# knagrecha/saturn

Hardware: NVIDIA H100
Metric: candidate schedules/sec (higher is better)
Workload: dtype f32

## Files before the change

saturn_b200/csrc/sb_common.cuh:

```cuda
#pragma once
#include <cuda_runtime.h>
#include <stdint.h>

#include "../../include/saturn_b200.h"

#if defined(__CUDA_ARCH__) && (__CUDA_ARCH__ != 900)
#error "saturn_b200 kernels target sm_90a (H100) only"
#endif

namespace sb {

constexpr int kSlots = SB_NSLOT;
constexpr int kWarp = 32;
constexpr int kMaxNodes = SB_MAX_NODES;
constexpr float kSentinel = 1.0e6f;

__device__ __forceinline__ float inf_f() { return __int_as_float(0x7f800000); }

__device__ __forceinline__ uint32_t smem_u32(const void* p) {
  return static_cast<uint32_t>(__cvta_generic_to_shared(p));
}
__device__ __forceinline__ uint32_t cluster_ctarank() {
  uint32_t r;
  asm volatile("mov.u32 %0, %%cluster_ctarank;" : "=r"(r));
  return r;
}
__device__ __forceinline__ void cluster_sync_all() {
  asm volatile("barrier.cluster.arrive.release.aligned;" ::: "memory");
  asm volatile("barrier.cluster.wait.acquire.aligned;" ::: "memory");
}
__device__ __forceinline__ uint32_t cluster_map_shared(uint32_t addr, uint32_t rank) {
  uint32_t r;
  asm volatile("mapa.shared::cluster.u32 %0, %1, %2;" : "=r"(r) : "r"(addr), "r"(rank));
  return r;
}

__device__ __forceinline__ void mbar_init(uint64_t* bar, uint32_t count) {
  asm volatile("mbarrier.init.shared::cta.b64 [%0], %1;" ::"r"(smem_u32(bar)), "r"(count) : "memory");
}
__device__ __forceinline__ void mbar_fence_init() {
  asm volatile("fence.mbarrier_init.release.cluster;" ::: "memory");
}
__device__ __forceinline__ void fence_proxy_async() {
  asm volatile("fence.proxy.async.shared::cta;" ::: "memory");
}
__device__ __forceinline__ void mbar_arrive_expect_tx(uint64_t* bar, uint32_t bytes) {
  asm volatile("mbarrier.arrive.expect_tx.shared::cta.b64 _, [%0], %1;" ::"r"(smem_u32(bar)), "r"(bytes)
               : "memory");
}
__device__ __forceinline__ bool mbar_try_wait(uint64_t* bar, uint32_t parity) {
  uint32_t ok;
  asm volatile(
      "{\n\t.reg .pred p;\n\t"
      "mbarrier.try_wait.parity.shared::cta.b64 p, [%1], %2;\n\t"
      "selp.u32 %0, 1, 0, p;\n\t}"
      : "=r"(ok)
      : "r"(smem_u32(bar)), "r"(parity)
      : "memory");
  return ok != 0;
}
__device__ __forceinline__ void mbar_wait(uint64_t* bar, uint32_t parity) {
  uint32_t spins = 0;
  while (!mbar_try_wait(bar, parity)) {
    if (++spins > (1u << 26)) __trap();
  }
}
__device__ __forceinline__ void tma_bulk_g2s(void* dst_smem, const void* src_gmem, uint32_t bytes,
                                             uint64_t* bar) {
  asm volatile(
      "cp.async.bulk.shared::cluster.global.mbarrier::complete_tx::bytes [%0], [%1], %2, [%3];" ::"r"(
          smem_u32(dst_smem)),
      "l"(src_gmem), "r"(bytes), "r"(smem_u32(bar))
      : "memory");
}

__device__ __forceinline__ void pmov_fma(float& dst, float src, int bit, int one) {
  int d = __float_as_int(dst);
  asm("{\n\t.reg .pred p;\n\tsetp.ne.s32 p, %2, 0;\n\t@p mad.lo.s32 %0, %1, %3, 0;\n\t}"
      : "+r"(d)
      : "r"(__float_as_int(src)), "r"(bit), "r"(one));
  dst = __int_as_float(d);
}
__device__ __forceinline__ void pinf_fma(float& dst, int bit) {
  asm("{\n\t.reg .pred p;\n\tsetp.ne.s32 p, %1, 0;\n\t@p add.f32 %0, %0, 0f7F800000;\n\t}" : "+f"(dst) : "r"(bit));
}
__device__ __forceinline__ float psel(float a, float b, int bit) {
  float r;
  asm("{\n\t.reg .pred p;\n\tsetp.ne.s32 p, %3, 0;\n\tselp.f32 %0, %1, %2, p;\n\t}" : "=f"(r) : "f"(a), "f"(b), "r"(bit));
  return r;
}

__device__ __forceinline__ float fmax3_mk(float mk, float b, float c) {
  return __int_as_float(__vimax3_s32(__float_as_int(mk), __float_as_int(b), __float_as_int(c)));
}

template <bool kIntegerStarts, bool kTrackMk = kIntegerStarts, bool kSum = false, bool kWeighted = false,
          bool kDue = false>
__device__ __forceinline__ void ls_step(float (&f)[8], float& mk, float& pend, float rt, int km1, int one, int ph,
                                        float w = 0.f, float d = 0.f) {
  static_assert(kSum || !kWeighted, "weights scale the sum of completion times only");
  static_assert(kWeighted || !kDue, "due dates run on the weighted form (unit weights for plain tardiness)");
  const float INF = inf_f();
  const int b2 = km1 & 4, b1 = km1 & 2, b0 = km1 & 1;
  float x0 = psel(f[4], f[0], b2), x1 = psel(f[5], f[1], b2), x2 = psel(f[6], f[2], b2), x3 = psel(f[7], f[3], b2);
  const float m2 = psel(INF, -0.0f, b2);
  float x4 = f[4] + m2, x5 = f[5] + m2, x6 = f[6] + m2, x7 = f[7] + m2;
  pmov_fma(x0, x2, b1, one); pmov_fma(x1, x3, b1, one); pmov_fma(x2, x4, b1, one); pmov_fma(x3, x5, b1, one);
  pmov_fma(x4, x6, b1, one); pmov_fma(x5, x7, b1, one); pinf_fma(x6, b1); pinf_fma(x7, b1);
  pmov_fma(x0, x1, b0, one); pmov_fma(x1, x2, b0, one); pmov_fma(x2, x3, b0, one); pmov_fma(x3, x4, b0, one);
  pmov_fma(x4, x5, b0, one); pmov_fma(x5, x6, b0, one); pmov_fma(x6, x7, b0, one); pinf_fma(x7, b0);
  const float s = x0;
  float v;
  if (kIntegerStarts) {
    v = s + ceilf(rt);
  } else {
    v = s + rt;
  }
  if (kSum) {
    const float e = kIntegerStarts ? s + rt : v;
    if (kDue) mk = __fadd_rn(mk, __fmul_rn(w, fmaxf(__fsub_rn(e, d), 0.f)));
    else if (kWeighted) mk = __fadd_rn(mk, __fmul_rn(w, e));
    else mk = mk + e;
  } else if (kTrackMk) {
    const float e = kIntegerStarts ? s + rt : v;
    if (ph < 0) mk = fmaxf(mk, e);
    else if (ph == 0) pend = e;
    else mk = fmax3_mk(mk, pend, e);
  }
  f[0] = fmaxf(f[0], fminf(v, x1));
  f[1] = fmaxf(f[1], fminf(v, x2));
  f[2] = fmaxf(f[2], fminf(v, x3));
  f[3] = fmaxf(f[3], fminf(v, x4));
  f[4] = fmaxf(f[4], fminf(v, x5));
  f[5] = fmaxf(f[5], fminf(v, x6));
  f[6] = fmaxf(f[6], fminf(v, x7));
  f[7] = fmaxf(f[7], v);
}

__device__ __forceinline__ unsigned long long pack_key(float mk, uint32_t id) {
  return (static_cast<unsigned long long>(__float_as_uint(mk)) << 32) | id;
}

__device__ __host__ __forceinline__ uint64_t mix64(uint64_t z) {
  z += 0x9e3779b97f4a7c15ull;
  z = (z ^ (z >> 30)) * 0xbf58476d1ce4e5b9ull;
  z = (z ^ (z >> 27)) * 0x94d049bb133111ebull;
  return z ^ (z >> 31);
}
__device__ __host__ __forceinline__ uint64_t rng_u64(uint64_t seed, uint64_t stream, uint64_t ctr) {
  return mix64(mix64(seed ^ (stream * 0xd1342543de82ef95ull)) + ctr * 0x2545f4914f6cdd1dull);
}

}
```

saturn_b200/csrc/sb_eval.cu:

```cuda
#include "sb_lane.cuh"

namespace sb {

struct TileArgs {
  const float* tab;
  int J, SG;
  const uint8_t* opt;
  const uint8_t* prio;
  long long B;
  long long stride_o, stride_p;
  int row_o, row_p;
  int copy_o, copy_p;
  int use_bulk;
  int nodes;
  float* out;
  unsigned long long* best_key;
  uint32_t id_base;
  long long ntiles;
  int one;
  SearchFuse sf;
  XchgPost xp;
  const float* w;
  const float* d;
};

template <int PB, bool INT, bool STREAM, bool MULTI, bool SEARCH = false, bool TABG = false, int ADDR = 0,
          bool SUM = false, bool W = false, bool D = false>
__global__ void __launch_bounds__(STREAM ? 512 : 384, 1) k_eval_tiles(const TileArgs a) {
  static_assert(!(SEARCH && (STREAM || TABG)), "the fused search round runs on shared-memory tiles only");
  static_assert(ADDR == 0 || (!TABG && !MULTI && !SEARCH), "ADDR = 1 needs the table and the opt rows in shared memory");
  static_assert(SUM || !W, "weights scale the sum of completion times only");
  static_assert(W || !D, "due dates run on the weighted form");
  extern __shared__ __align__(128) uint8_t smem[];
  const int nw = blockDim.x >> 5;
  const int warp = threadIdx.x >> 5, lane = threadIdx.x & 31;
  const uint32_t tab_bytes = TABG ? 0u : static_cast<uint32_t>(a.J) * a.SG * 4u;
  const uint32_t w_bytes = (W && !TABG) ? ((static_cast<uint32_t>(a.J) * 4u + 15u) & ~15u) : 0u;
  const uint32_t d_bytes = D ? w_bytes : 0u;
  float* tab_s = reinterpret_cast<float*>(smem);
  [[maybe_unused]] float* w_s = reinterpret_cast<float*>(smem + tab_bytes);
  [[maybe_unused]] float* d_s = reinterpret_cast<float*>(smem + tab_bytes + w_bytes);
  uint64_t* bars = reinterpret_cast<uint64_t*>(smem + ((tab_bytes + w_bytes + d_bytes + 15u) & ~15u));
  uint8_t* tiles = reinterpret_cast<uint8_t*>(bars) + (((1 + nw) * 8 + 15) & ~15);
  const uint32_t node_bytes = MULTI ? static_cast<uint32_t>(a.nodes) * 1024u : 0u;
  const uint32_t tile_bytes = 32u * (a.row_o + (STREAM ? 0 : a.row_p)) + node_bytes;
  uint8_t* wbase = tiles + static_cast<size_t>(warp) * tile_bytes;
  float4* node_s = reinterpret_cast<float4*>(wbase);
  uint8_t* tile_o = wbase + node_bytes;
  uint8_t* tile_p = tile_o + 32u * a.row_o;
  uint64_t* bar_tab = bars;
  uint64_t* bar_w = bars + 1 + warp;

  if (threadIdx.x == 0) {
    mbar_init(bar_tab, 1);
    for (int w = 0; w < nw; ++w) mbar_init(bars + 1 + w, 1);
    mbar_fence_init();
  }
  __syncthreads();
  if constexpr (!TABG) {
    if (threadIdx.x == 0) {
      mbar_arrive_expect_tx(bar_tab, tab_bytes + w_bytes + d_bytes);
      const uint8_t* src = reinterpret_cast<const uint8_t*>(a.tab);
      for (uint32_t off = 0; off < tab_bytes; off += 32768u) {
        uint32_t n = min(32768u, tab_bytes - off);
        tma_bulk_g2s(smem + off, src + off, n, bar_tab);
      }
      if constexpr (W) {
        const uint8_t* wsrc = reinterpret_cast<const uint8_t*>(a.w);
        for (uint32_t off = 0; off < w_bytes; off += 32768u)
          tma_bulk_g2s(smem + tab_bytes + off, wsrc + off, min(32768u, w_bytes - off), bar_tab);
      }
      if constexpr (D) {
        const uint8_t* dsrc = reinterpret_cast<const uint8_t*>(a.d);
        for (uint32_t off = 0; off < d_bytes; off += 32768u)
          tma_bulk_g2s(smem + tab_bytes + w_bytes + off, dsrc + off, min(32768u, d_bytes - off), bar_tab);
      }
    }
  }

  LaneState<INT, MULTI, ADDR, SUM, (W ? (TABG ? 2 : 1) : 0), D> st;
  if (TABG) st.tab = a.tab;
  else st.tab = tab_s;
  if constexpr (W) {
    st.wt = TABG ? a.w : w_s;
    st.wt_s = smem_u32(w_s);
  }
  if constexpr (D) {
    st.dd = TABG ? a.d : d_s;
    st.dd_s = smem_u32(d_s);
  }
  st.SG = a.SG;
  st.one = a.one;
  st.orow = tile_o + lane * a.row_o;
  st.ns = node_s + lane;
  st.orow_s = smem_u32(tile_o + lane * a.row_o);
  st.tab_s = smem_u32(tab_s);
  st.four = static_cast<uint32_t>(a.one) * 4u;

  bool fold_pending = a.xp.counter != nullptr && a.xp.fold_prev && a.xp.seq > 1 && blockIdx.x == 0 && warp == 0;
  unsigned long long pf_seen = 0ull, pf_key = ~0ull;
  auto look_issue = [&]() {
    if (lane < a.xp.x.world) {
      const unsigned long long* slot = a.xp.x.peer[lane] + ((a.xp.seq - 1) & 1ull) * 2;
      asm volatile("ld.acquire.sys.global.u64 %0, [%1];" : "=l"(pf_seen) : "l"(slot + 1) : "memory");
      asm volatile("ld.relaxed.sys.global.u64 %0, [%1];" : "=l"(pf_key) : "l"(slot) : "memory");
    }
  };
  auto fold_keys = [&](unsigned long long k) {
#pragma unroll
    for (int d = 16; d > 0; d >>= 1) {
      const unsigned long long o = __shfl_xor_sync(0xffffffffu, k, d);
      k = o < k ? o : k;
    }
    if (lane == 0) atomicMin(a.best_key, k);
    fold_pending = false;
  };
  auto look_consume = [&]() {
    const unsigned long long want = a.xp.seq - 1;
    const bool ok = lane >= a.xp.x.world || pf_seen >= want;
    if (__all_sync(0xffffffffu, ok)) fold_keys(lane < a.xp.x.world ? pf_key : ~0ull);
  };
  auto try_fold = [&](bool block) {
    const unsigned long long want = a.xp.seq - 1;
    unsigned long long k = ~0ull;
    bool ok = true;
    if (lane < a.xp.x.world) {
      const unsigned long long* slot = a.xp.x.peer[lane] + (want & 1ull) * 2;
      unsigned long long seen;
      unsigned spins = 0;
      for (;;) {
        asm volatile("ld.acquire.sys.global.u64 %0, [%1];" : "=l"(seen) : "l"(slot + 1) : "memory");
        if (seen >= want || !block || ++spins >= (1u << 22)) break;
        __nanosleep(64);
      }
      ok = seen >= want;
      if (ok) asm volatile("ld.relaxed.sys.global.u64 %0, [%1];" : "=l"(k) : "l"(slot) : "memory");
    }
    ok = __all_sync(0xffffffffu, ok);
    if (!ok) {
      if (block && lane == 0) *a.xp.error = 1;
      return;
    }
    fold_keys(k);
  };
  if (fold_pending) look_issue();

  uint32_t phase = 0;
  bool tab_ready = TABG;
  for (long long tile = static_cast<long long>(blockIdx.x) * nw + warp; tile < a.ntiles;
       tile += static_cast<long long>(gridDim.x) * nw) {
    const long long b0 = tile * 32;
    if (!SEARCH && fold_pending) {
      look_consume();
      if (fold_pending) look_issue();
    }
    const long long cand = (SEARCH && a.sf.deal) ? lane * a.ntiles + tile : b0 + lane;
    const bool active = cand < a.B;
    const int nb = SEARCH ? __popc(__ballot_sync(0xffffffffu, active)) : static_cast<int>(min(32ll, a.B - b0));
    const uint8_t* pg = a.prio + cand * a.stride_p;
    __syncwarp();
    PrioChunk q;
    if (a.use_bulk) {
      fence_proxy_async();
      if (lane == 0)
        mbar_arrive_expect_tx(bar_w, static_cast<uint32_t>(nb) * (a.copy_o + (STREAM ? 0 : a.copy_p)));
      __syncwarp();
      if (active) {
        tma_bulk_g2s(tile_o + lane * a.row_o, a.opt + cand * a.stride_o, a.copy_o, bar_w);
        if (!STREAM) tma_bulk_g2s(tile_p + lane * a.row_p, pg, a.copy_p, bar_w);
      }
      if (STREAM && active) q = ld_prio32<true>(pg);
      mbar_wait(bar_w, phase);
      phase ^= 1;
    } else {
      for (int r = 0; r < nb; ++r) {
        const uint8_t* so = a.opt + (b0 + r) * a.stride_o;
        const uint8_t* sp = a.prio + (b0 + r) * a.stride_p;
        for (int x = lane; x < a.J; x += 32) tile_o[r * a.row_o + x] = so[x];
        for (int x = lane; x < a.J * PB; x += 32) tile_p[r * a.row_p + x] = sp[x];
      }
      __syncwarp();
    }
    if (!tab_ready) {
      mbar_wait(bar_tab, 0);
      tab_ready = true;
    }
    auto evaluate = [&](const uint8_t* prio_row_s) -> float {
      st.reset(a.nodes);
      const int J = a.J;
      if constexpr (STREAM && ADDR == 1) {
        constexpr int STEPS = 32;
        constexpr int kBatch = 8;
        const int nch = (J + STEPS - 1) / STEPS, nfull = J / STEPS;
        uint32_t ob[kBatch];
        float rb[kBatch];
        [[maybe_unused]] float wb[kBatch];
        [[maybe_unused]] float db[kBatch];
        auto resolve = [&](const uint32_t* w) {
          int js[kBatch];
#pragma unroll
          for (int i = 0; i < kBatch; ++i) js[i] = prio_at<1>(w, i);
#pragma unroll
          for (int i = 0; i < kBatch; ++i) ob[i] = st.gather_opt(js[i]);
#pragma unroll
          for (int i = 0; i < kBatch; ++i) rb[i] = st.gather_rt(js[i], ob[i]);
          if constexpr (W) {
#pragma unroll
            for (int i = 0; i < kBatch; ++i) wb[i] = st.gather_w(js[i]);
          }
          if constexpr (D) {
#pragma unroll
            for (int i = 0; i < kBatch; ++i) db[i] = st.gather_d(js[i]);
          }
        };
        if (nfull > 0) resolve(q.w);
        for (int c = 0; c < nfull; ++c) {
          PrioChunk nxt = q;
          if (c + 1 < nch) nxt = ld_prio32<true>(pg + (c + 1) * 32);
          const bool ahead = c + 1 < nfull;
          uint32_t head[kBatch / 4];
#pragma unroll
          for (int i = 0; i < kBatch / 4; ++i) head[i] = ahead ? nxt.w[i] : q.w[i];
#pragma unroll
          for (int b = 0; b < STEPS / kBatch; ++b) {
            uint32_t oc[kBatch];
            float rc[kBatch];
            [[maybe_unused]] float wc[kBatch];
            [[maybe_unused]] float dc[kBatch];
#pragma unroll
            for (int i = 0; i < kBatch; ++i) { oc[i] = ob[i]; rc[i] = rb[i]; }
            if constexpr (W) {
#pragma unroll
              for (int i = 0; i < kBatch; ++i) wc[i] = wb[i];
            }
            if constexpr (D) {
#pragma unroll
              for (int i = 0; i < kBatch; ++i) dc[i] = db[i];
            }
            resolve(b + 1 < STEPS / kBatch ? q.w + (b + 1) * (kBatch / 4) : head);
#pragma unroll
            for (int i = 0; i < kBatch; ++i) {
              if constexpr (D) st.step_resolved(static_cast<int>(oc[i]), rc[i], i & 1, wc[i], dc[i]);
              else if constexpr (W) st.step_resolved(static_cast<int>(oc[i]), rc[i], i & 1, wc[i]);
              else st.step_resolved(static_cast<int>(oc[i]), rc[i], i & 1);
            }
          }
          q = nxt;
        }
        if (nfull < nch) {
          const int rem = J - nfull * STEPS;
#pragma unroll
          for (int t = 0; t < STEPS; ++t)
            if (t < rem) st.step(prio_at<1>(q.w, t), t & 1);
        }
      } else if (STREAM) {
        constexpr int STEPS = 32 / PB;
        const int nch = (J + STEPS - 1) / STEPS;
        for (int c = 0; c < nch; ++c) {
          PrioChunk nxt = q;
          if (c + 1 < nch) nxt = ld_prio32<true>(pg + (c + 1) * 32);
          if ((c + 1) * STEPS <= J) {
#pragma unroll
            for (int t = 0; t < STEPS; ++t) st.step(prio_at<PB>(q.w, t), t & 1);
          } else {
            const int rem = J - c * STEPS;
#pragma unroll
            for (int t = 0; t < STEPS; ++t)
              if (t < rem) st.step(prio_at<PB>(q.w, t), t & 1);
          }
          q = nxt;
        }
      } else {
        const uint4* prow = reinterpret_cast<const uint4*>(prio_row_s);
        constexpr int STEPS = 16 / PB;
        const int nch = (J + STEPS - 1) / STEPS;
        for (int c = 0; c < nch; ++c) {
          const uint4 p = prow[c];
          const uint32_t w[4] = {p.x, p.y, p.z, p.w};
          if ((c + 1) * STEPS <= J) {
#pragma unroll
            for (int t = 0; t < STEPS; ++t) st.step(prio_at<PB>(w, t), t & 1);
          } else {
            const int rem = J - c * STEPS;
#pragma unroll
            for (int t = 0; t < STEPS; ++t)
              if (t < rem) st.step(prio_at<PB>(w, t), t & 1);
          }
        }
// ... 308 lines not shown
    for (int g = 0; g < a.nodes * kSlots; ++g) ready[g] = 0.f;
    float mk = 0.f;
    for (int i = 0; i < a.J; ++i) {
      const int j = PB == 1 ? prow[i] : reinterpret_cast<const uint16_t*>(prow)[i];
      const int o = orow[j];
      const int k = (o & 7) + 1;
      const int node = multi ? (o >> 3) : 0;
      const float rt = __ldg(a.tab + static_cast<size_t>(j) * a.SG + (multi ? (o & 7) : o));
      float* rd = ready + node * kSlots;
      uint32_t taken = 0;
      float s = 0.f;
      for (int q = 0; q < k; ++q) {
        int best = -1;
        float bv = 0.f;
        for (int g = 0; g < kSlots; ++g) {
          const bool free_slot = ((taken >> g) & 1u) == 0u;
          if (free_slot && (best < 0 || rd[g] < bv)) {
            best = g;
            bv = rd[g];
          }
        }
        taken |= 1u << best;
        s = bv;
      }
      const float hold = (INT && isfinite(rt)) ? ceilf(rt) : rt;
      const float nxt = s + hold;
      for (int g = 0; g < kSlots; ++g)
        if ((taken >> g) & 1u) rd[g] = nxt;
      if constexpr (D)
        mk = __fadd_rn(mk, __fmul_rn(__ldg(a.w + j), fmaxf(__fsub_rn(s + rt, __ldg(a.d + j)), 0.f)));
      else if constexpr (W) mk = __fadd_rn(mk, __fmul_rn(__ldg(a.w + j), s + rt));
      else if (SUM) mk = mk + (s + rt);
      else mk = fmaxf(mk, s + rt);
      if (a.start) a.start[b * a.J + j] = s;
      if (a.slotmask) a.slotmask[b * a.J + j] = (static_cast<uint32_t>(node) << 16) | taken;
    }
    if (a.out) a.out[b] = mk;
  }
}

__global__ void k_validate(const float* tab, int J, int SG, int nodes, const uint8_t* opt, const uint8_t* prio, int pb,
                           long long B, long long stride_o, long long stride_p, unsigned long long* bad, int by_pos) {
  const int lane = threadIdx.x & 31;
  const long long warp = (static_cast<long long>(blockIdx.x) * blockDim.x + threadIdx.x) >> 5;
  const long long nwarps = (static_cast<long long>(gridDim.x) * blockDim.x) >> 5;
  extern __shared__ uint32_t seen_all[];
  const int words = (J + 31) / 32;
  uint32_t* seen = seen_all + (threadIdx.x >> 5) * words;
  for (long long b = warp; b < B; b += nwarps) {
    for (int w = lane; w < words; w += 32) seen[w] = 0;
    __syncwarp();
    bool ok = true;
    const uint8_t* orow = opt + b * stride_o;
    const uint8_t* prow = prio + b * stride_p;
    for (int i = lane; i < J; i += 32) {
      const int j = pb == 1 ? prow[i] : reinterpret_cast<const uint16_t*>(prow)[i];
      if (j >= J) {
        ok = false;
      } else {
        const uint32_t old = atomicOr(&seen[j >> 5], 1u << (j & 31));
        if (old & (1u << (j & 31))) ok = false;
      }
      int o = orow[i];
      if (nodes > 1) {
        if ((o >> 3) >= nodes) ok = false;
        o &= 7;
      }
      const int job = by_pos ? (j < J ? j : 0) : i;
      if (o >= SG || !isfinite(tab[static_cast<size_t>(job) * SG + o])) ok = false;
    }
    ok = __all_sync(0xffffffffu, ok);
    if (!ok && lane == 0) atomicAdd(bad, 1ull);
    __syncwarp();
  }
}

static int round_row(int bytes) {
  int r16 = (bytes + 15) / 16;
  if ((r16 & 1) == 0) r16 += 1;
  return r16 * 16;
}

int plan_tiles(const Device& dev, int J, int SG, int pb, bool stream, int nodes, TilePlan* tp, bool tab_global,
               int arrays) {
  tp->row_o = round_row(J);
  tp->row_p = round_row(J * pb);
  tp->copy_o = (J + 15) & ~15;
  tp->copy_p = (J * pb + 15) & ~15;
  size_t tab_bytes = tab_global ? 0 : ((static_cast<size_t>(J) * SG * 4 + 15) & ~size_t(15));
  if (!tab_global) tab_bytes += arrays * job_array_bytes(J);
  const size_t per_warp = 32u * static_cast<size_t>(tp->row_o + (stream ? 0 : tp->row_p)) +
                          (nodes > 1 ? static_cast<size_t>(nodes) * 1024u : 0u);
  int nw = stream ? 16 : 12;
  while (nw > 0 && tab_bytes + 16 * ((1 + nw + 1) / 2) + nw * per_warp > dev.smem_optin) --nw;
  tp->warps = nw;
  tp->smem = tab_bytes + (((1 + nw) * 8 + 15) & ~15) + nw * per_warp;
  return nw;
}

using TileKernel = void (*)(TileArgs);

static bool bulk_aligned(const EvalCall& c) {
  return (c.stride_o % 16 == 0) && (c.stride_p % 16 == 0) && (reinterpret_cast<uintptr_t>(c.opt) % 16 == 0) &&
         (reinterpret_cast<uintptr_t>(c.prio) % 16 == 0);
}

static TileArgs tile_args(const EvalCall& c, const TilePlan& tp) {
  TileArgs a;
  a.tab = c.tab; a.J = c.J; a.SG = c.SG; a.opt = c.opt; a.prio = c.prio; a.B = c.B;
  a.stride_o = c.stride_o; a.stride_p = c.stride_p;
  a.row_o = tp.row_o; a.row_p = tp.row_p; a.copy_o = tp.copy_o; a.copy_p = tp.copy_p;
  a.nodes = c.nodes;
  a.out = c.out; a.best_key = c.best_key; a.id_base = c.id_base;
  a.w = c.w;
  a.d = c.d;
  a.ntiles = (c.B + 31) / 32;
  a.one = 1;
  return a;
}

static cudaError_t launch_tiles(const Device& dev, TileKernel kern, const TileArgs& a, const TilePlan& tp,
                                cudaStream_t st) {
  long long ctas = (a.ntiles + tp.warps - 1) / tp.warps;
  int grid = static_cast<int>(ctas < dev.sm_count ? ctas : dev.sm_count);
  return launch(kern, grid, tp.warps * 32, tp.smem, st, a);
}

cudaError_t eval_launch(const Device& dev, const EvalCall& c, cudaStream_t st, int* path_used) {
  if (c.B <= 0) return cudaSuccess;
  const int pb = c.J <= 256 ? 1 : 2;
  const bool multi = c.nodes > 1;
  const bool bulk_ok = bulk_aligned(c);
  const bool stream_ok = bulk_ok && (c.stride_p % 32 == 0) && (reinterpret_cast<uintptr_t>(c.prio) % 32 == 0) &&
                         !(c.flags & HOOK_NO_STREAM);
  const int arrays = job_arrays(c.flags);
  TilePlan tp;
  int nw = 0;
  bool stream = false, tabg = false;
  if (!c.force_generic) {
    if (stream_ok) {
      nw = plan_tiles(dev, c.J, c.SG, pb, true, c.nodes, &tp, false, arrays);
      stream = nw >= 2 && c.stride_o >= tp.copy_o && c.stride_p >= ((c.J * pb + 31) & ~31);
      if (!stream && !multi) {
        nw = plan_tiles(dev, c.J, c.SG, pb, true, c.nodes, &tp, true);
        stream = tabg = nw >= 2 && c.stride_o >= tp.copy_o && c.stride_p >= ((c.J * pb + 31) & ~31);
      }
    }
    if (!stream) nw = plan_tiles(dev, c.J, c.SG, pb, false, c.nodes, &tp, false, arrays);
  }
  if (nw >= 2) {
    TileArgs a = tile_args(c, tp);
    a.use_bulk = stream || (bulk_ok && (c.stride_o >= tp.copy_o) && (c.stride_p >= tp.copy_p));
    a.xp = c.xp;
    if (path_used) *path_used = tabg ? 4 : (stream ? 3 : (a.use_bulk ? 2 : 1));
    const bool fma_addr = pb == 1 && stream && !tabg && !multi && !(c.flags & HOOK_PLAIN_ADDR);
    const TileKernel kern = with_eval_types(pb, c.flags, [&](auto PB, auto INT, auto SUM, auto W, auto D) -> TileKernel {
      if (tabg) return k_eval_tiles<PB, INT, true, false, false, true, 0, SUM, W, D>;
      if constexpr (PB == 1) {
        if (fma_addr) return k_eval_tiles<1, INT, true, false, false, false, 1, SUM, W, D>;
      }
      return with_bool(stream, [&](auto STREAM) {
        return with_bool(multi, [&](auto MULTI) -> TileKernel {
          return k_eval_tiles<PB, INT, STREAM, MULTI, false, false, 0, SUM, W, D>;
        });
      });
    });
    return launch_tiles(dev, kern, a, tp, st);
  }
  GenericArgs g;
  g.tab = c.tab; g.J = c.J; g.SG = c.SG; g.opt = c.opt; g.prio = c.prio; g.B = c.B;
  g.stride_o = c.stride_o; g.stride_p = c.stride_p; g.out = c.out; g.best_key = c.best_key;
  g.id_base = c.id_base; g.tab_in_smem = 0; g.nodes = c.nodes; g.one = 1; g.w = c.w; g.d = c.d;
  if (path_used) *path_used = 0;
  const size_t tab_bytes = static_cast<size_t>(c.J) * c.SG * 4;
  size_t smem = multi ? static_cast<size_t>(4) * c.nodes * 1024u : 0u;
  if (tab_bytes <= dev.smem_optin / 2) {
    g.tab_in_smem = 1;
    smem += tab_bytes;
  }
  long long blocks = (c.B + 127) / 128;
  long long cap = static_cast<long long>(dev.sm_count) * 8;
  int grid = static_cast<int>(blocks < cap ? blocks : cap);
  if (grid < 1) grid = 1;
  const auto kern = with_eval_types(pb, c.flags, [&](auto PB, auto INT, auto SUM, auto W, auto D) {
    return with_bool(multi, [&](auto MULTI) { return k_eval_generic<PB, INT, MULTI, SUM, W, D>; });
  });
  return launch(kern, grid, 128, smem, st, g);
}

int search_round_mode(const Device& dev, int J, int SG, int nodes, int arrays) {
  const int pb = J <= 256 ? 1 : 2;
  TilePlan tp;
  return plan_tiles(dev, J, SG, pb, false, nodes, &tp, false, arrays) >= 8 ? 2 : 0;
}

cudaError_t search_round_launch(const Device& dev, const EvalCall& c, const SearchFuse& sf, cudaStream_t st) {
  if (c.B <= 0) return cudaSuccess;
  const int pb = c.J <= 256 ? 1 : 2;
  TilePlan tp;
  const int arrays = job_arrays(c.flags);
  if (search_round_mode(dev, c.J, c.SG, c.nodes, arrays) == 0 || !bulk_aligned(c)) return cudaErrorNotSupported;
  plan_tiles(dev, c.J, c.SG, pb, false, c.nodes, &tp, false, arrays);
  if (c.stride_o < tp.copy_o || c.stride_p < tp.copy_p) return cudaErrorNotSupported;
  TileArgs a = tile_args(c, tp);
  a.use_bulk = 1;
  a.sf = sf;
  const TileKernel kern = with_eval_types(pb, c.flags, [&](auto PB, auto INT, auto SUM, auto W, auto D) {
    return with_bool(c.nodes > 1, [&](auto MULTI) -> TileKernel {
      return k_eval_tiles<PB, INT, false, MULTI, true, false, 0, SUM, W, D>;
    });
  });
  return launch_tiles(dev, kern, a, tp, st);
}

cudaError_t eval_full_launch(const Device& dev, const EvalCall& c, float* start, uint32_t* slotmask, cudaStream_t st) {
  if (c.B <= 0) return cudaSuccess;
  const int pb = c.J <= 256 ? 1 : 2;
  FullArgs a;
  a.tab = c.tab; a.J = c.J; a.SG = c.SG; a.opt = c.opt; a.prio = c.prio; a.B = c.B;
  a.stride_o = c.stride_o; a.stride_p = c.stride_p; a.nodes = c.nodes < 1 ? 1 : c.nodes;
  a.out = c.out; a.start = start; a.slotmask = slotmask; a.w = c.w; a.d = c.d;
  long long blocks = (c.B + 127) / 128;
  long long cap = static_cast<long long>(dev.sm_count) * 16;
  int grid = static_cast<int>(blocks < cap ? blocks : cap);
  const auto kern = with_eval_types(pb, c.flags, [](auto PB, auto INT, auto SUM, auto W, auto D) {
    return k_eval_full<PB, INT, SUM, W, D>;
  });
  return launch(kern, grid, 128, 0, st, a);
}

cudaError_t validate_launch(const Device& dev, const EvalCall& c, unsigned long long* bad, cudaStream_t st, bool by_pos) {
  if (c.B <= 0) return cudaSuccess;
  const int pb = c.J <= 256 ? 1 : 2;
  const int words = (c.J + 31) / 32;
  const int threads = 128;
  size_t smem = static_cast<size_t>(threads / 32) * words * 4;
  long long blocks = (c.B + 3) / 4;
  long long cap = static_cast<long long>(dev.sm_count) * 8;
  int grid = static_cast<int>(blocks < cap ? blocks : cap);
  k_validate<<<grid, threads, smem, st>>>(c.tab, c.J, c.SG, c.nodes, c.opt, c.prio, pb, c.B, c.stride_o, c.stride_p, bad,
                                          by_pos ? 1 : 0);
// ... 5 lines not shown
```

saturn_b200/csrc/sb_internal.h:

```cpp
#pragma once
#include <cuda_runtime.h>
#include <stdint.h>

#include <type_traits>

#include "sb_common.cuh"

namespace sb {

enum : unsigned {
  HOOK_FORCE_GENERIC = 0x80000000u,
  HOOK_NO_STREAM = 0x40000000u,
  HOOK_NO_FUSED = 0x20000000u,
  HOOK_NO_INCREMENTAL = 0x10000000u,
  HOOK_VERIFY_INCREMENTAL = 0x08000000u,
  HOOK_ROUND1_MOVES = 0x04000000u,
  HOOK_PLAIN_ADDR = 0x02000000u,
  HOOK_WINDOW_BIAS = 0x01000000u,
  HOOK_TABLE_GLOBAL = 0x00800000u,
  HOOK_TABLE_PAIR = 0x00400000u,
  HOOK_REORDER = 0x00200000u,
  HOOK_NO_REORDER = 0x00100000u,
};
static_assert(((HOOK_FORCE_GENERIC | HOOK_NO_STREAM | HOOK_NO_FUSED | HOOK_NO_INCREMENTAL | HOOK_VERIFY_INCREMENTAL |
// ... 41 lines not shown
    if (e != cudaSuccess) return e;
  }
  kern<<<grid, block, smem, st>>>(args...);
  return cudaGetLastError();
}

struct Device {
  int ordinal = 0;
  int sm_count = 0;
  size_t smem_optin = 0;
};

constexpr int kMaxRanks = 16;
struct XchgDev {
  int rank = 0, world = 1;
  unsigned long long* local = nullptr;
  unsigned long long* peer[kMaxRanks] = {nullptr};
};
struct XchgPost {
  XchgDev x;
  unsigned long long seq = 0;
  unsigned* counter = nullptr;
  int fold_prev = 0;
  int* error = nullptr;
};
cudaError_t xchg_post_launch(const XchgDev& x, const unsigned long long* key, unsigned long long seq, cudaStream_t st);
cudaError_t xchg_reduce_launch(const XchgDev& x, unsigned long long seq, unsigned long long* out,
                               unsigned long long* fold, int* error, cudaStream_t st);
cudaError_t xchg_post_reduce_launch(const XchgDev& x, const unsigned long long* key, unsigned long long seq,
                                    unsigned long long* out , cudaStream_t st);

struct TilePlan {
  int warps = 0;
  int row_o = 0, row_p = 0, copy_o = 0, copy_p = 0;
  size_t smem = 0;
};

struct EvalCall {
  const float* tab = nullptr;
  const float* w = nullptr;
  const float* d = nullptr;
  int J = 0, SG = 0;
  const uint8_t* opt = nullptr;
  const uint8_t* prio = nullptr;
  long long B = 0;
  long long stride_o = 0, stride_p = 0;
  unsigned flags = 0;
  int nodes = 1;
  float* out = nullptr;
  unsigned long long* best_key = nullptr;
  uint32_t id_base = 0;
  int force_generic = 0;
  XchgPost xp;
};

constexpr int kMaxFusedRounds = 16;
constexpr int kSnapPos = 32;
struct SearchFuse {
  float* cur_mk = nullptr;
  uint8_t* cur_o = nullptr;
  uint8_t* cur_p = nullptr;
  const uint8_t* vopt = nullptr;
  const int* nvalid = nullptr;
  uint64_t seed = 0, chain_base = 0;
  int round = 0;
  int nrounds = 1;
  int nodes = 1;
  float temperature[kMaxFusedRounds] = {};
  int resample_every = 0;
  int deal = 0;
  int win = 0;
  int win_bias = 0;
  float* snap = nullptr;
  unsigned long long* verify_bad = nullptr;
  struct KeepBest {
    unsigned* counter = nullptr;
    unsigned long long* keys = nullptr;
    uint8_t *best_o = nullptr, *best_p = nullptr;
    long long chains = 0, stride_o = 0, stride_p = 0;
  } keep;
};

int plan_tiles(const Device& dev, int J, int SG, int pb, bool stream, int nodes, TilePlan* tp, bool tab_global = false,
               int arrays = 0);
cudaError_t eval_launch(const Device& dev, const EvalCall& c, cudaStream_t st, int* path_used);
cudaError_t eval_alt_launch(const Device& dev, const EvalCall& c, cudaStream_t st);
int search_round_mode(const Device& dev, int J, int SG, int nodes, int arrays = 0);
cudaError_t search_round_launch(const Device& dev, const EvalCall& c, const SearchFuse& sf, cudaStream_t st);
cudaError_t eval_full_launch(const Device& dev, const EvalCall& c, float* start, uint32_t* slotmask, cudaStream_t st);
cudaError_t validate_launch(const Device& dev, const EvalCall& c, unsigned long long* bad, cudaStream_t st,
                            bool by_pos = false);

cudaError_t build_table_launch(const float* T, int J, int S, int G, uint64_t gcount_packed, float* tab, float* tmin,
                               uint8_t* args, cudaStream_t st);
cudaError_t build_valid_launch(const float* tmin, const uint8_t* args, int J, int reduced, float sentinel, uint8_t* vopt,
                               int* nvalid, cudaStream_t st);

}
```

saturn_b200/csrc/sb_lane.cuh:

```cuda
#pragma once
#include "sb_internal.h"

namespace sb {

struct PrioChunk {
  uint32_t w[8];
};
template <bool kReadOnly>
__device__ __forceinline__ PrioChunk ld_prio32(const uint8_t* p) {
  PrioChunk c;
  if (kReadOnly) {
    asm volatile("ld.global.nc.L1::no_allocate.v4.u32 {%0,%1,%2,%3}, [%8];\n\t"
                 "ld.global.nc.L1::no_allocate.v4.u32 {%4,%5,%6,%7}, [%8+16];"
                 : "=r"(c.w[0]), "=r"(c.w[1]), "=r"(c.w[2]), "=r"(c.w[3]), "=r"(c.w[4]), "=r"(c.w[5]), "=r"(c.w[6]),
                   "=r"(c.w[7])
                 : "l"(p));
  } else {
    asm volatile("ld.global.L1::no_allocate.v4.u32 {%0,%1,%2,%3}, [%8];\n\t"
                 "ld.global.L1::no_allocate.v4.u32 {%4,%5,%6,%7}, [%8+16];"
                 : "=r"(c.w[0]), "=r"(c.w[1]), "=r"(c.w[2]), "=r"(c.w[3]), "=r"(c.w[4]), "=r"(c.w[5]), "=r"(c.w[6]),
                   "=r"(c.w[7])
                 : "l"(p)
                 : "memory");
  }
  return c;
}

template <bool INT, bool MULTI, int ADDR = 0, bool SUM = false, int WGT = 0, bool DUE = false>
struct LaneState {
  float f[8];
  float mk;
  float pend;
  const uint8_t* orow;
  const float* tab;
  const float* wt;
  const float* dd;
  int SG;
  int one;
  uint32_t orow_s, tab_s, four;
  uint32_t wt_s;
  uint32_t dd_s;
  float4* ns;
  int cur;

  __device__ __forceinline__ void reset(int nodes) {
#pragma unroll
    for (int i = 0; i < 8; ++i) f[i] = 0.f;
    mk = 0.f;
    pend = 0.f;
    cur = 0;
    if (MULTI) {
      const float4 z = make_float4(0.f, 0.f, 0.f, 0.f);
      for (int n = 0; n < 2 * nodes; ++n) ns[n * 32] = z;
    }
  }
  __device__ __forceinline__ void switch_node(int n) {
    if (n != cur) {
      float4* old = ns + (2 * cur) * 32;
      old[0] = make_float4(f[0], f[1], f[2], f[3]);
      old[32] = make_float4(f[4], f[5], f[6], f[7]);
      const float4* slot = ns + (2 * n) * 32;
      const float4 lo = slot[0], hi = slot[32];
      f[0] = lo.x; f[1] = lo.y; f[2] = lo.z; f[3] = lo.w;
      f[4] = hi.x; f[5] = hi.y; f[6] = hi.z; f[7] = hi.w;
      cur = n;
    }
  }
  __device__ __forceinline__ int lookup_opt(int j) const { return orow[j]; }
  __device__ __forceinline__ float lookup_rt(int j, int o) const {
    return MULTI ? tab[j * 8 + (o & 7)] : tab[j * SG + o];
  }
  __device__ __forceinline__ float lookup_w(int j) const {
    if constexpr (WGT == 1) return wt[j];
    else if constexpr (WGT == 2) return __ldg(wt + j);
    else return 0.f;
  }
  __device__ __forceinline__ float lookup_d(int j) const {
    if constexpr (!DUE) return 0.f;
    else if constexpr (WGT == 1) return dd[j];
    else return __ldg(dd + j);
  }
  __device__ __forceinline__ void step_resolved(int o, float rt, int ph = -1, float w = 0.f, float d = 0.f) {
    if (!MULTI) {
      ls_step<INT, INT, SUM, (WGT != 0), DUE>(f, mk, pend, rt, o & 7, one, ph, w, d);
    } else {
      switch_node(o >> 3);
      ls_step<INT, true, SUM, (WGT != 0), DUE>(f, mk, pend, rt, o & 7, one, ph, w, d);
    }
  }
  __device__ __forceinline__ uint32_t gather_opt(int j) const {
    uint32_t oa, o;
    asm("mad.lo.u32 %0, %1, %2, %3;" : "=r"(oa) : "r"(j), "r"(one), "r"(orow_s));
    asm("ld.shared.u8 %0, [%1];" : "=r"(o) : "r"(oa));
    return o;
  }
  __device__ __forceinline__ float gather_rt(int j, uint32_t o) const {
    uint32_t idx, ta;
    float rt;
    asm("mad.lo.u32 %0, %1, %2, %3;" : "=r"(idx) : "r"(j), "r"(SG), "r"(o));
    asm("mad.lo.u32 %0, %1, %2, %3;" : "=r"(ta) : "r"(idx), "r"(four), "r"(tab_s));
    asm("ld.shared.f32 %0, [%1];" : "=f"(rt) : "r"(ta));
    return rt;
  }
  __device__ __forceinline__ float gather_w(int j) const {
    if constexpr (WGT == 0) {
      return 0.f;
    } else {
      uint32_t wa;
      float w;
      asm("mad.lo.u32 %0, %1, %2, %3;" : "=r"(wa) : "r"(j), "r"(four), "r"(wt_s));
      asm("ld.shared.f32 %0, [%1];" : "=f"(w) : "r"(wa));
      return w;
    }
  }
  __device__ __forceinline__ float gather_d(int j) const {
    if constexpr (!DUE) {
      return 0.f;
    } else {
      uint32_t da;
      float d;
      asm("mad.lo.u32 %0, %1, %2, %3;" : "=r"(da) : "r"(j), "r"(four), "r"(dd_s));
      asm("ld.shared.f32 %0, [%1];" : "=f"(d) : "r"(da));
      return d;
    }
  }
  __device__ __forceinline__ void step(int j, int ph = -1) {
    constexpr bool W = WGT != 0;
    if (!MULTI && ADDR == 1) {
      const uint32_t o = gather_opt(j);
      ls_step<INT, INT, SUM, W, DUE>(f, mk, pend, gather_rt(j, o), static_cast<int>(o & 7u), one, ph, gather_w(j),
                                     gather_d(j));
      return;
    }
    const int o = orow[j];
    if (!MULTI) {
      const float rt = tab[j * SG + o];
      ls_step<INT, INT, SUM, W, DUE>(f, mk, pend, rt, o & 7, one, ph, lookup_w(j), lookup_d(j));
    } else {
      const int col = o & 7;
      const float rt = tab[j * 8 + col];
      switch_node(o >> 3);
      ls_step<INT, true, SUM, W, DUE>(f, mk, pend, rt, col, one, ph, lookup_w(j), lookup_d(j));
    }
  }
  __device__ __forceinline__ float result() const { return SUM ? mk : ((INT || MULTI) ? fmaxf(mk, pend) : f[7]); }
  __device__ __forceinline__ float running() const { return SUM ? mk : fmaxf(mk, pend); }
};

template <int PB>
__device__ __forceinline__ int prio_at(const uint32_t* w, int t) {
  if (PB == 1) return static_cast<int>(__byte_perm(w[t >> 2], 0u, 0x4440u + (t & 3)));
  return static_cast<int>(__byte_perm(w[t >> 1], 0u, (t & 1) ? 0x4432u : 0x4410u));
}

__device__ __forceinline__ bool fold_best(unsigned long long* best_key, bool active, float mk, uint32_t id, int lane) {
  const uint32_t bits = active ? __float_as_uint(mk) : 0xffffffffu;
  const uint32_t mn = __reduce_min_sync(0xffffffffu, bits);
  const uint32_t who = __ballot_sync(0xffffffffu, bits == mn);
  bool lowered = false;
  if (lane == __ffs(who) - 1 && active) {
    const unsigned long long key = pack_key(mk, id);
    if (key < *reinterpret_cast<volatile unsigned long long*>(best_key)) lowered = key < atomicMin(best_key, key);
  }
  return lowered;
}

__device__ __forceinline__ uint32_t launch_incumbent_bits(const SearchFuse& sf) {
  return sf.keep.keys != nullptr
             ? static_cast<uint32_t>(*reinterpret_cast<volatile unsigned long long*>(sf.keep.keys + 1) >> 32)
             : 0u;
}

__device__ __forceinline__ void keep_best_tail(const SearchFuse& sf) {
  __threadfence();
  __syncthreads();
  int mine = 0;
  if (threadIdx.x == 0) {
    const unsigned done = atomicAdd(sf.keep.counter, 1u);
    mine = done == gridDim.x - 1;
    if (mine) *sf.keep.counter = 0;
  }
  if (!__syncthreads_or(mine) || threadIdx.x >= 32) return;
  __threadfence();
  const int lane = threadIdx.x;
  const unsigned long long key = *reinterpret_cast<volatile unsigned long long*>(sf.keep.keys);
  if ((key >> 32) >= (*reinterpret_cast<volatile unsigned long long*>(sf.keep.keys + 1) >> 32)) return;
  const long long c = static_cast<long long>(((key & 0xffffffffull) - (sf.chain_base & 0xffffffffull)) & 0xffffffffull);
  if (c >= sf.keep.chains) return;
  const uint4* so = reinterpret_cast<const uint4*>(sf.cur_o + c * sf.keep.stride_o);
  const uint4* sp = reinterpret_cast<const uint4*>(sf.cur_p + c * sf.keep.stride_p);
  for (int i = lane; i * 16 < sf.keep.stride_o; i += 32) reinterpret_cast<uint4*>(sf.keep.best_o)[i] = __ldcg(so + i);
  for (int i = lane; i * 16 < sf.keep.stride_p; i += 32) reinterpret_cast<uint4*>(sf.keep.best_p)[i] = __ldcg(sp + i);
  __syncwarp();
  if (lane == 0) sf.keep.keys[1] = key;
}

struct Move {
  int kind;
  int a, b;
  int va, vb;
};

__device__ __forceinline__ uint32_t bounded32(uint64_t r, uint32_t n) {
  return static_cast<uint32_t>((static_cast<uint64_t>(static_cast<uint32_t>(r >> 32)) * n) >> 32);
}

template <int PB>
__device__ __forceinline__ int smem_prio_ld(const uint8_t* row, int i) {
  return PB == 1 ? row[i] : reinterpret_cast<const uint16_t*>(row)[i];
}
// ... 185 lines not shown
```

Baseline: 1.963 billion.

## Resolve job table addresses with byte_perm on pre-scaled opt rows

Adds an ADDR=2 path for the streamed single-priority kernel when SG is 64. Each lane's opt row is padded to 256 bytes and 256-byte aligned, then pre-multiplied by four in shared memory so a single __byte_perm can build both the opt and runtime-table addresses straight from the packed u8 prio word. This drops the per-step multiply-add address arithmetic and the byte extraction, and ls_step reads its selector bits from shifted positions. In exchange it uses more shared memory per warp, adds a per-tile scaling pass, and relies on a fixed layout that only holds when the job count and SG fit into byte-wide offsets.

New measurement: 2.029 billion, median of 6. +3.3%, better.

```diff
diff --git a/saturn_b200/csrc/sb_common.cuh b/saturn_b200/csrc/sb_common.cuh
--- a/saturn_b200/csrc/sb_common.cuh
+++ b/saturn_b200/csrc/sb_common.cuh
@@ -95,13 +95,13 @@
 }
 
 template <bool kIntegerStarts, bool kTrackMk = kIntegerStarts, bool kSum = false, bool kWeighted = false,
-          bool kDue = false>
+          bool kDue = false, int kKBit = 0>
 __device__ __forceinline__ void ls_step(float (&f)[8], float& mk, float& pend, float rt, int km1, int one, int ph,
                                         float w = 0.f, float d = 0.f) {
   static_assert(kSum || !kWeighted, "weights scale the sum of completion times only");
   static_assert(kWeighted || !kDue, "due dates run on the weighted form (unit weights for plain tardiness)");
   const float INF = inf_f();
-  const int b2 = km1 & 4, b1 = km1 & 2, b0 = km1 & 1;
+  const int b2 = km1 & (4 << kKBit), b1 = km1 & (2 << kKBit), b0 = km1 & (1 << kKBit);
   float x0 = psel(f[4], f[0], b2), x1 = psel(f[5], f[1], b2), x2 = psel(f[6], f[2], b2), x3 = psel(f[7], f[3], b2);
   const float m2 = psel(INF, -0.0f, b2);
   float x4 = f[4] + m2, x5 = f[5] + m2, x6 = f[6] + m2, x7 = f[7] + m2;
diff --git a/saturn_b200/csrc/sb_eval.cu b/saturn_b200/csrc/sb_eval.cu
--- a/saturn_b200/csrc/sb_eval.cu
+++ b/saturn_b200/csrc/sb_eval.cu
@@ -29,6 +29,7 @@
 __global__ void __launch_bounds__(STREAM ? 512 : 384, 1) k_eval_tiles(const TileArgs a) {
   static_assert(!(SEARCH && (STREAM || TABG)), "the fused search round runs on shared-memory tiles only");
   static_assert(ADDR == 0 || (!TABG && !MULTI && !SEARCH), "ADDR = 1 needs the table and the opt rows in shared memory");
+  static_assert(ADDR != 2 || (PB == 1 && STREAM), "ADDR = 2 takes the job ids from streamed u8 prio words");
   static_assert(SUM || !W, "weights scale the sum of completion times only");
   static_assert(W || !D, "due dates run on the weighted form");
   extern __shared__ __align__(128) uint8_t smem[];
@@ -42,6 +43,7 @@
   [[maybe_unused]] float* d_s = reinterpret_cast<float*>(smem + tab_bytes + w_bytes);
   uint64_t* bars = reinterpret_cast<uint64_t*>(smem + ((tab_bytes + w_bytes + d_bytes + 15u) & ~15u));
   uint8_t* tiles = reinterpret_cast<uint8_t*>(bars) + (((1 + nw) * 8 + 15) & ~15);
+  if constexpr (ADDR == 2) tiles += (0u - smem_u32(tiles)) & 255u;
   const uint32_t node_bytes = MULTI ? static_cast<uint32_t>(a.nodes) * 1024u : 0u;
   const uint32_t tile_bytes = 32u * (a.row_o + (STREAM ? 0 : a.row_p)) + node_bytes;
   uint8_t* wbase = tiles + static_cast<size_t>(warp) * tile_bytes;
@@ -96,6 +98,7 @@
   st.orow_s = smem_u32(tile_o + lane * a.row_o);
   st.tab_s = smem_u32(tab_s);
   st.four = static_cast<uint32_t>(a.one) * 4u;
+  st.tabb = smem;
 
   bool fold_pending = a.xp.counter != nullptr && a.xp.fold_prev && a.xp.seq > 1 && blockIdx.x == 0 && warp == 0;
   unsigned long long pf_seen = 0ull, pf_key = ~0ull;
@@ -181,6 +184,18 @@
       }
       __syncwarp();
     }
+    if constexpr (ADDR == 2) {
+      if (active) {
+        uint4* row = reinterpret_cast<uint4*>(tile_o + lane * a.row_o);
+        auto x4 = [&](uint32_t& x) { asm("mad.lo.u32 %0, %0, %1, 0;" : "+r"(x) : "r"(st.four)); };
+#pragma unroll
+        for (int i = 0; i < 16; ++i) {
+          uint4 v = row[(i + lane) & 15];
+          x4(v.x); x4(v.y); x4(v.z); x4(v.w);
+          row[(i + lane) & 15] = v;
+        }
+      }
+    }
     if (!tab_ready) {
       mbar_wait(bar_tab, 0);
       tab_ready = true;
@@ -188,7 +203,7 @@
     auto evaluate = [&](const uint8_t* prio_row_s) -> float {
       st.reset(a.nodes);
       const int J = a.J;
-      if constexpr (STREAM && ADDR == 1) {
+      if constexpr (STREAM && ADDR >= 1) {
         constexpr int STEPS = 32;
         constexpr int kBatch = 8;
         const int nch = (J + STEPS - 1) / STEPS, nfull = J / STEPS;
@@ -197,13 +212,22 @@
         [[maybe_unused]] float wb[kBatch];
         [[maybe_unused]] float db[kBatch];
         auto resolve = [&](const uint32_t* w) {
-          int js[kBatch];
-#pragma unroll
-          for (int i = 0; i < kBatch; ++i) js[i] = prio_at<1>(w, i);
-#pragma unroll
-          for (int i = 0; i < kBatch; ++i) ob[i] = st.gather_opt(js[i]);
-#pragma unroll
-          for (int i = 0; i < kBatch; ++i) rb[i] = st.gather_rt(js[i], ob[i]);
+          [[maybe_unused]] int js[kBatch];
+          if constexpr (ADDR == 1 || W) {
+#pragma unroll
+            for (int i = 0; i < kBatch; ++i) js[i] = prio_at<1>(w, i);
+          }
+          if constexpr (ADDR == 2) {
+#pragma unroll
+            for (int i = 0; i < kBatch; ++i) ob[i] = st.gather_opt(w[i >> 2], i & 3);
+#pragma unroll
+            for (int i = 0; i < kBatch; ++i) rb[i] = st.gather_rt(w[i >> 2], i & 3, ob[i]);
+          } else {
+#pragma unroll
+            for (int i = 0; i < kBatch; ++i) ob[i] = st.gather_opt(js[i]);
+#pragma unroll
+            for (int i = 0; i < kBatch; ++i) rb[i] = st.gather_rt(js[i], ob[i]);
+          }
           if constexpr (W) {
 #pragma unroll
             for (int i = 0; i < kBatch; ++i) wb[i] = st.gather_w(js[i]);
@@ -678,13 +702,14 @@
 }
 
 int plan_tiles(const Device& dev, int J, int SG, int pb, bool stream, int nodes, TilePlan* tp, bool tab_global,
-               int arrays) {
-  tp->row_o = round_row(J);
+               int arrays, bool perm_rows) {
+  tp->row_o = perm_rows ? 256 : round_row(J);
   tp->row_p = round_row(J * pb);
   tp->copy_o = (J + 15) & ~15;
   tp->copy_p = (J * pb + 15) & ~15;
   size_t tab_bytes = tab_global ? 0 : ((static_cast<size_t>(J) * SG * 4 + 15) & ~size_t(15));
   if (!tab_global) tab_bytes += arrays * job_array_bytes(J);
+  if (perm_rows) tab_bytes += 240;
   const size_t per_warp = 32u * static_cast<size_t>(tp->row_o + (stream ? 0 : tp->row_p)) +
                           (nodes > 1 ? static_cast<size_t>(nodes) * 1024u : 0u);
   int nw = stream ? 16 : 12;
@@ -744,15 +769,24 @@
     }
     if (!stream) nw = plan_tiles(dev, c.J, c.SG, pb, false, c.nodes, &tp, false, arrays);
   }
+  const bool fma_addr = nw >= 2 && pb == 1 && stream && !tabg && !multi && !(c.flags & HOOK_PLAIN_ADDR);
+  bool perm = false;
+  if (fma_addr && c.SG == 64 && !(c.flags & SB_FLAG_DUE)) {
+    TilePlan tpp;
+    perm = plan_tiles(dev, c.J, c.SG, pb, true, c.nodes, &tpp, false, arrays, true) >= nw;
+    if (perm) tp = tpp;
+  }
   if (nw >= 2) {
     TileArgs a = tile_args(c, tp);
     a.use_bulk = stream || (bulk_ok && (c.stride_o >= tp.copy_o) && (c.stride_p >= tp.copy_p));
     a.xp = c.xp;
     if (path_used) *path_used = tabg ? 4 : (stream ? 3 : (a.use_bulk ? 2 : 1));
-    const bool fma_addr = pb == 1 && stream && !tabg && !multi && !(c.flags & HOOK_PLAIN_ADDR);
     const TileKernel kern = with_eval_types(pb, c.flags, [&](auto PB, auto INT, auto SUM, auto W, auto D) -> TileKernel {
       if (tabg) return k_eval_tiles<PB, INT, true, false, false, true, 0, SUM, W, D>;
       if constexpr (PB == 1) {
+        if constexpr (!D) {
+          if (perm) return k_eval_tiles<1, INT, true, false, false, false, 2, SUM, W, false>;
+        }
         if (fma_addr) return k_eval_tiles<1, INT, true, false, false, false, 1, SUM, W, D>;
       }
       return with_bool(stream, [&](auto STREAM) {
diff --git a/saturn_b200/csrc/sb_internal.h b/saturn_b200/csrc/sb_internal.h
--- a/saturn_b200/csrc/sb_internal.h
+++ b/saturn_b200/csrc/sb_internal.h
@@ -147,7 +147,7 @@
 };
 
 int plan_tiles(const Device& dev, int J, int SG, int pb, bool stream, int nodes, TilePlan* tp, bool tab_global = false,
-               int arrays = 0);
+               int arrays = 0, bool perm_rows = false);
 cudaError_t eval_launch(const Device& dev, const EvalCall& c, cudaStream_t st, int* path_used);
 cudaError_t eval_alt_launch(const Device& dev, const EvalCall& c, cudaStream_t st);
 int search_round_mode(const Device& dev, int J, int SG, int nodes, int arrays = 0);
diff --git a/saturn_b200/csrc/sb_lane.cuh b/saturn_b200/csrc/sb_lane.cuh
--- a/saturn_b200/csrc/sb_lane.cuh
+++ b/saturn_b200/csrc/sb_lane.cuh
@@ -35,6 +35,7 @@
   const float* tab;
   const float* wt;
   const float* dd;
+  const uint8_t* tabb;
   int SG;
   int one;
   uint32_t orow_s, tab_s, four;
@@ -81,7 +82,9 @@
     else return __ldg(dd + j);
   }
   __device__ __forceinline__ void step_resolved(int o, float rt, int ph = -1, float w = 0.f, float d = 0.f) {
-    if (!MULTI) {
+    if (ADDR == 2) {
+      ls_step<INT, INT, SUM, (WGT != 0), DUE, 2>(f, mk, pend, rt, o, one, ph, w, d);
+    } else if (!MULTI) {
       ls_step<INT, INT, SUM, (WGT != 0), DUE>(f, mk, pend, rt, o & 7, one, ph, w, d);
     } else {
       switch_node(o >> 3);
@@ -101,6 +104,16 @@
     asm("mad.lo.u32 %0, %1, %2, %3;" : "=r"(ta) : "r"(idx), "r"(four), "r"(tab_s));
     asm("ld.shared.f32 %0, [%1];" : "=f"(rt) : "r"(ta));
     return rt;
+  }
+  __device__ __forceinline__ uint32_t gather_opt(uint32_t pw, int t) const {
+    const uint32_t oa = __byte_perm(pw, orow_s, 0x7650u + t);
+    uint32_t o4;
+    asm("ld.shared.u8 %0, [%1];" : "=r"(o4) : "r"(oa));
+    return o4;
+  }
+  __device__ __forceinline__ float gather_rt(uint32_t pw, int t, uint32_t o4) const {
+    const uint32_t off = __byte_perm(pw, o4, 0x5504u | (t << 4));
+    return *reinterpret_cast<const float*>(tabb + off);
   }
   __device__ __forceinline__ float gather_w(int j) const {
     if constexpr (WGT == 0) {
@@ -126,6 +139,12 @@
   }
   __device__ __forceinline__ void step(int j, int ph = -1) {
     constexpr bool W = WGT != 0;
+    if (ADDR == 2) {
+      const uint32_t o4 = gather_opt(static_cast<uint32_t>(j), 0);
+      ls_step<INT, INT, SUM, W, DUE, 2>(f, mk, pend, gather_rt(static_cast<uint32_t>(j), 0, o4), static_cast<int>(o4),
+                                        one, ph, gather_w(j), gather_d(j));
+      return;
+    }
     if (!MULTI && ADDR == 1) {
       const uint32_t o = gather_opt(j);
       ls_step<INT, INT, SUM, W, DUE>(f, mk, pend, gather_rt(j, o), static_cast<int>(o & 7u), one, ph, gather_w(j),
```
